# Amano-Ginji/distributed-tensorflow-example

Hardware: AMD Instinct MI355X
Metric: samples/sec (whole node) MNIST MLP sync-SGD at 1/2/4/8 MI355X; step-time p50 (higher is better)
Workload: dtype fp32; 1 GPU; model=mlp-784-100-10 (example.py), global_batch=100, per_gpu_batch=100, parallelism=dp1, optimizer=sgd lr=0.0005, grad_allreduce=none, engine=persistent-fp32, exchange_mode=persistent, launch=single process, steps_per_launch=550, hipgraph_steps=0, input_prefetch=in-kernel copier workgroups, activation=sigmoid

## Files before the change

csrc/kernels/mlp_persist_f32.hip:

```cpp
#include "common.h"
#include "mlp_api.h"

#include <atomic>

#include <cstdlib>

namespace dtfk {
namespace mlpf {

typedef __attribute__((ext_vector_type(4))) uint32_t u32x4;
typedef __attribute__((address_space(1))) unsigned gu32;

constexpr int DIN = 784, HID = 100, NCLS = 10;
constexpr int NJ = 7;
constexpr int NQ = 4;
constexpr int NTW = 2;
constexpr int NBT = 7;
constexpr int BROWS = 16 * NBT;
constexpr int XTS = 128;
constexpr int NCOMP = NJ * NQ;
constexpr int THREADS = 512;
constexpr int NCOP = 16;
constexpr int NCOPR = 14;
constexpr int RES_LR_BYTE = 124;
// ... 257 lines not shown
  f32x4 S0 = {0.f, 0.f, 0.f, 0.f}, S1 = S0;
#pragma unroll
  for (int r0 = 0; r0 < NW; r0 += GRP) {
    if (r0 >= W) break;
    u32x4 v0[GRP], v1[GRP];
#pragma unroll
    for (int i = 0; i < GRP; ++i) {
      const int r = r0 + i;
      const bool on = r < W && r != rank && hv;
      const auto rs = prs.r[r];
      if constexpr (BF) {
        if constexpr (TWO) {
          v0[i] = __builtin_amdgcn_raw_buffer_load_b128(rs, on ? so + e0 : OOB_OFF, 0, SYS);
        } else {
          const u32x2 h = __builtin_amdgcn_raw_buffer_load_b64(rs, on ? so + e0 : OOB_OFF, 0, SYS);
          v0[i] = u32x4{h[0], h[1], 0u, 0u};
        }
      } else {
        v0[i] = __builtin_amdgcn_raw_buffer_load_b128(rs, on ? so + e0 : OOB_OFF, 0, SYS);
        if constexpr (TWO) v1[i] = __builtin_amdgcn_raw_buffer_load_b128(rs, on ? so + e1 : OOB_OFF, 0, SYS);
      }
    }
#pragma unroll
    for (int i = 0; i < GRP; ++i) {
      const int r = r0 + i;
      if (r >= W) break;
      const bool me = r == rank;
      f32x4 P0, P1 = {0.f, 0.f, 0.f, 0.f};
      if constexpr (BF) {
        P0 = unbf4(v0[i][0], v0[i][1]);
        if constexpr (TWO) P1 = unbf4(v0[i][2], v0[i][3]);
      } else {
        P0 = __builtin_bit_cast(f32x4, v0[i]);
        if constexpr (TWO) P1 = __builtin_bit_cast(f32x4, v1[i]);
      }
      S0 += me ? G0 : P0;
      S1 += me ? G1 : P1;
    }
  }
  G0 = S0;
  G1 = S1;
}
template <int NW>
__device__ __forceinline__ void sum_small(const PeerRs<NW>& prs, int W, int rank, int so, bool dlane, bool blane,
                                          int lane, f32x4& D, float& gb) {
  u32x4 d[NW];
  uint32_t b[NW];
#pragma unroll
  for (int r = 0; r < NW; ++r) {
    const bool on = r < W && r != rank;
    const auto rs = prs.r[r];
    d[r] = __builtin_amdgcn_raw_buffer_load_b128(rs, (on && dlane) ? so + lane * 16 : OOB_OFF, 0, SYS);
    b[r] = __builtin_amdgcn_raw_buffer_load_b32(rs, (on && blane) ? so + 1024 + lane * 4 : OOB_OFF, 0, SYS);
  }
  f32x4 SD = {0.f, 0.f, 0.f, 0.f};
  float SB = 0.f;
#pragma unroll
  for (int r = 0; r < NW; ++r) {
    if (r >= W) break;
    const bool me = r == rank;
    SD += me ? D : __builtin_bit_cast(f32x4, d[r]);
    SB += me ? gb : __uint_as_float(b[r]);
  }
  D = SD;
  gb = SB;
}

__device__ void copier(const Args& a, int cid, uint8_t* smem) {
  const int tid = threadIdx.x;
  const int B = a.B;
  if (tid == 0) { PRO(NCOMP + cid, 0); }
  for (int st = cid; st < a.next_steps; st += NCOP) {
    const uint8_t* src = a.host_next + (long long)st * a.rec_h;
    uint8_t* dst = a.stage_next + (long long)st * REC;
    constexpr int C16 = DIN / 16;
    for (int k = tid; k < BROWS * C16; k += THREADS) {
      const int row = k / C16, c = k % C16;
      uint4 v = make_uint4(0u, 0u, 0u, 0u);
      if (row < B) v = reinterpret_cast<const uint4*>(src)[row * C16 + c];
      *reinterpret_cast<uint4*>(smem + row * CROW + 16 * c) = v;
    }
    if (tid < 128) dst[XROW_BYTES + XT_BYTES + tid] = tid < B ? src[(long long)B * DIN + tid] : (uint8_t)0;
    __syncthreads();
    for (int k = tid; k < BROWS * C16; k += THREADS) {
      const int row = k / C16, c = k % C16;
      reinterpret_cast<uint4*>(dst)[row * C16 + c] = *reinterpret_cast<const uint4*>(smem + row * CROW + 16 * c);
    }
    uint8_t* xt = dst + XROW_BYTES;
    for (int k = tid; k < (DIN / 4) * (BROWS / 4); k += THREADS) {
      const int fq = k / (BROWS / 4), rq = k % (BROWS / 4);
      const uint8_t* p = smem + 4 * rq * CROW + 4 * fq;
      const uint32_t r0 = *reinterpret_cast<const uint32_t*>(p);
      const uint32_t r1 = *reinterpret_cast<const uint32_t*>(p + CROW);
      const uint32_t r2 = *reinterpret_cast<const uint32_t*>(p + 2 * CROW);
      const uint32_t r3 = *reinterpret_cast<const uint32_t*>(p + 3 * CROW);
      const uint32_t t01 = __builtin_amdgcn_perm(r1, r0, 0x05010400u);
      const uint32_t t23 = __builtin_amdgcn_perm(r3, r2, 0x05010400u);
      const uint32_t u01 = __builtin_amdgcn_perm(r1, r0, 0x07030602u);
      const uint32_t u23 = __builtin_amdgcn_perm(r3, r2, 0x07030602u);
      uint32_t* o = reinterpret_cast<uint32_t*>(xt + (long long)(4 * fq) * XTS + 4 * rq);
      o[0] = __builtin_amdgcn_perm(t23, t01, 0x05040100u);
      o[XTS / 4] = __builtin_amdgcn_perm(t23, t01, 0x07060302u);
      o[2 * XTS / 4] = __builtin_amdgcn_perm(u23, u01, 0x05040100u);
      o[3 * XTS / 4] = __builtin_amdgcn_perm(u23, u01, 0x07060302u);
    }
    __syncthreads();
  }
  if (tid == 0) { PRO(NCOMP + cid, 1); }
}

__device__ void copier_res(const Args& a, int cid, uint8_t* smem) {
  if (cid >= NCOPR) return;
  const int tid = threadIdx.x;
  constexpr int RR = 8;
  int* dec = reinterpret_cast<int*>(smem + RR * CROW);
  const int B = a.B;
  const int hb = (int)(2 * a.rec_h);
  const auto hrs = __builtin_amdgcn_make_buffer_rsrc(const_cast<uint8_t*>(a.host_recs), 0, hb, 0x00020000);
  for (int st = 0;; ++st) {
    const long long k = a.run0 + st;
    if (tid == 0) {
      int d = 1;
      const long long t0 = (long long)__builtin_amdgcn_s_memrealtime();
      const long long lim = cid == 0 ? a.idle : a.idle + a.timeout;
      for (;;) {
        const long long v = __hip_atomic_load(a.door, __ATOMIC_RELAXED, __HIP_MEMORY_SCOPE_SYSTEM);
        if (v < 0) { d = 0; break; }
        if (v > k) break;
        if (cid != 0 && __hip_atomic_load(a.dctr + 16, __ATOMIC_RELAXED, __HIP_MEMORY_SCOPE_AGENT) != 0u) { d = 0; break; }
        if ((long long)__builtin_amdgcn_s_memrealtime() - t0 > lim) { d = 0; break; }
        __builtin_amdgcn_s_sleep(1);
      }
      if (cid == 0 && !d) __hip_atomic_store(a.dctr + 16, 1u, __ATOMIC_RELAXED, __HIP_MEMORY_SCOPE_AGENT);
      if (cid == 0 && d) { RTS(k, 0); }
      *dec = d;
    }
    __syncthreads();
    if (*dec == 0) break;
    const int slot = (int)(k & 1);
    const int hbase = slot * (int)a.rec_h;
    const int r0 = RR * cid;
    uint8_t* dst = const_cast<uint8_t*>(a.stage) + (long long)(st & 1) * REC;
    constexpr int C16 = DIN / 16;
    constexpr int NLD = (RR * C16 + THREADS - 1) / THREADS;
    u32x4 hv[NLD];
    uint32_t lv = 0;
    if (cid == 0 && tid < 32) {
      if (4 * tid == RES_LR_BYTE)
        lv = __float_as_uint(__hip_atomic_load(a.host_lr + slot, __ATOMIC_RELAXED, __HIP_MEMORY_SCOPE_SYSTEM));
      else
        lv = __builtin_amdgcn_raw_buffer_load_b32(hrs, 4 * tid < B ? hbase + B * DIN + 4 * tid : OOB_OFF, 0, SYS);
    }
#pragma unroll
    for (int i = 0; i < NLD; ++i) {
      const int t = tid + i * THREADS;
      const int rr = t / C16, cc = t % C16;
      const int row = r0 + rr;
      hv[i] = __builtin_amdgcn_raw_buffer_load_b128(hrs, (t < RR * C16 && row < B) ? hbase + row * DIN + 16 * cc : OOB_OFF,
                                                    0, SYS);
    }
#pragma unroll
    for (int i = 0; i < NLD; ++i) {
      const int t = tid + i * THREADS;
      if (t < RR * C16) *reinterpret_cast<u32x4*>(smem + (t / C16) * CROW + 16 * (t % C16)) = hv[i];
    }
    __syncthreads();
    for (int t = tid; t < RR * C16; t += THREADS) {
      const int rr = t / C16, cc = t % C16;
      const u32x4 v = *reinterpret_cast<const u32x4*>(smem + rr * CROW + 16 * cc);
      __builtin_amdgcn_raw_buffer_store_b128(v, region_rsrc(dst, (int)REC), (r0 + rr) * DIN + 16 * cc, 0, 16);
    }
    for (int t = tid; t < (DIN / 4) * (RR / 4); t += THREADS) {
      const int fq = t >> 1, rq = t & 1;
      const uint8_t* p = smem + 4 * rq * CROW + 4 * fq;
      const uint32_t q0 = *reinterpret_cast<const uint32_t*>(p);
      const uint32_t q1 = *reinterpret_cast<const uint32_t*>(p + CROW);
      const uint32_t q2 = *reinterpret_cast<const uint32_t*>(p + 2 * CROW);
      const uint32_t q3 = *reinterpret_cast<const uint32_t*>(p + 3 * CROW);
      const uint32_t t01 = __builtin_amdgcn_perm(q1, q0, 0x05010400u);
      const uint32_t t23 = __builtin_amdgcn_perm(q3, q2, 0x05010400u);
      const uint32_t u01 = __builtin_amdgcn_perm(q1, q0, 0x07030602u);
      const uint32_t u23 = __builtin_amdgcn_perm(q3, q2, 0x07030602u);
      const auto rs = region_rsrc(dst, (int)REC);
      const int o = (int)XROW_BYTES + (4 * fq) * XTS + r0 + 4 * rq;
      __builtin_amdgcn_raw_buffer_store_b32(__builtin_amdgcn_perm(t23, t01, 0x05040100u), rs, o, 0, 16);
      __builtin_amdgcn_raw_buffer_store_b32(__builtin_amdgcn_perm(t23, t01, 0x07060302u), rs, o + XTS, 0, 16);
      __builtin_amdgcn_raw_buffer_store_b32(__builtin_amdgcn_perm(u23, u01, 0x05040100u), rs, o + 2 * XTS, 0, 16);
      __builtin_amdgcn_raw_buffer_store_b32(__builtin_amdgcn_perm(u23, u01, 0x07060302u), rs, o + 3 * XTS, 0, 16);
    }
    if (cid == 0 && tid < 32) {
      uint32_t v = lv;
      if (4 * tid != RES_LR_BYTE) {
        const int nv = B - 4 * tid;
        if (nv < 4) v = nv <= 0 ? 0u : (v & ((1u << (8 * nv)) - 1u));
      }
      __builtin_amdgcn_raw_buffer_store_b32(v, region_rsrc(dst, (int)REC), (int)(XROW_BYTES + XT_BYTES) + 4 * tid, 0,
                                            16);
    }
    asm volatile("s_waitcnt vmcnt(0)" ::: "memory");
    __syncthreads();
    if (tid == 0) {
      __hip_atomic_fetch_add(a.dctr, 1u, __ATOMIC_RELAXED, __HIP_MEMORY_SCOPE_AGENT);
      if (cid == 0) { RTS(k, 1); }
    }
  }
  if (cid == 0 && tid == 0)
    __hip_atomic_store(a.host_state, a.launch_id, __ATOMIC_RELAXED, __HIP_MEMORY_SCOPE_SYSTEM);
}

template <int ACT, int NW, bool SPLIT, bool RES, bool INS = false>
__device__ void compute(const Args& a, const int j, const int q, uint8_t* smem) {
  const int dbg = INS ? a.dbg : 0;
  constexpr bool MULTI = NW > 1;
  const int tid = threadIdx.x, lane = tid & 63, w = __builtin_amdgcn_readfirstlane(tid >> 6);
  const int r = lane & 15, g = lane >> 4;
  const int c = j * NQ + q;
  const int B = a.B;
  f32x4* zbuf = reinterpret_cast<f32x4*>(smem + L_ZBUF);
  float* a2T = reinterpret_cast<float*>(smem + L_A2T);
  float* dz2T = reinterpret_cast<float*>(smem + L_DZ2T);
  float* dz3T = reinterpret_cast<float*>(smem + L_DZ3T);
  float* w2s = reinterpret_cast<float*>(smem + L_W2);
  float* b1s = reinterpret_cast<float*>(smem + L_B1);
  float* b2s = reinterpret_cast<float*>(smem + L_B2);
  float* rdb2 = reinterpret_cast<float*>(smem + L_RDB2);
  int* abort_flag = reinterpret_cast<int*>(smem + L_FLAG);
  int* census = abort_flag + 1;
  uint16_t* dzp = reinterpret_cast<uint16_t*>(smem + L_DZP);
  if (tid == 0) { PROC(c, 0); }

  const int hid = 16 * j + r;
  const bool hv = hid < HID;
  const int nt = ntile(q);
  const bool tv0 = w < nt, tv1 = w + 8 < nt;
  const int ft0 = tile0(q) + w, ft1 = tile0(q) + (tv1 ? w + 8 : 0);
  auto tvk = [=](int k) { return k ? tv1 : tv0; };
  auto ftk = [=](int k) { return k ? ft1 : ft0; };
  float Wt[NTW][4];
  f32x4 wld[NTW];
  if constexpr (RES) {
#pragma unroll
    for (int k = 0; k < NTW; ++k)
#pragma unroll
      for (int e = 0; e < 4; ++e)
        Wt[k][e] = (tvk(k) && hv) ? a.params[(16 * ftk(k) + 4 * g + e) * HID + hid] : 0.f;
  } else if constexpr (MULTI) {
    const int u0 = 16 * j + 4 * (r & 3);
#pragma unroll
    for (int k = 0; k < NTW; ++k)
      wld[k] = (tvk(k) && u0 < HID)
                   ? *reinterpret_cast<const f32x4*>(a.params + (16 * ftk(k) + 4 * g + (r >> 2)) * HID + u0)
                   : f32x4{0.f, 0.f, 0.f, 0.f};
  } else {
    const int u0 = 16 * j + 4 * (r & 3);
    const auto rw1 = __builtin_amdgcn_make_buffer_rsrc(a.params, 0, DIN * HID * 4, 0x00020000);
#pragma unroll
    for (int k = 0; k < NTW; ++k)
      wld[k] = __builtin_bit_cast(
          f32x4, __builtin_amdgcn_raw_buffer_load_b128(
                     rw1, (tvk(k) && u0 < HID) ? ((16 * ftk(k) + 4 * g + (r >> 2)) * HID + u0) * 4 : OOB_OFF, 0, 0));
  }
  float pv = 0.f;
  if constexpr (MULTI) {
    if (tid < 256) {
      const int n = tid >> 4, cl = tid & 15;
      const int hn = 16 * j + n;
      pv = (hn < HID && cl < NCLS) ? a.p_w2[hn * NCLS + cl] : 0.f;
    } else if (tid < 272) {
      const int hn = 16 * j + (tid - 256);
      pv = hn < HID ? a.p_b1[hn] : 0.f;
    } else if (tid < 288) {
      const int cl = tid - 272;
      pv = cl < NCLS ? a.p_b2[cl] : 0.f;
    }
  } else {
    const int n = tid >> 4, cl = tid & 15, hn = 16 * j + n, hb = 16 * j + (tid - 256), c2 = tid - 272;
    const auto rw2 = __builtin_amdgcn_make_buffer_rsrc(a.p_w2, 0, HID * NCLS * 4, 0x00020000);
    const auto rb1 = __builtin_amdgcn_make_buffer_rsrc(a.p_b1, 0, HID * 4, 0x00020000);
    const auto rb2 = __builtin_amdgcn_make_buffer_rsrc(a.p_b2, 0, NCLS * 4, 0x00020000);
    const uint32_t v0 =
        __builtin_amdgcn_raw_buffer_load_b32(rw2, (tid < 256 && hn < HID && cl < NCLS) ? (hn * NCLS + cl) * 4 : OOB_OFF, 0, 0);
    const uint32_t v1 =
        __builtin_amdgcn_raw_buffer_load_b32(rb1, (tid >= 256 && tid < 272 && hb < HID) ? hb * 4 : OOB_OFF, 0, 0);
    const uint32_t v2 =
        __builtin_amdgcn_raw_buffer_load_b32(rb2, (tid >= 272 && tid < 288 && c2 < NCLS) ? c2 * 4 : OOB_OFF, 0, 0);
    pv = __uint_as_float(v0 | v1 | v2);
  }
  unsigned long long seq0 = *a.seq;
  long long gstep0 = *a.gstep;
  float lr = *a.lr;
  const unsigned xcc = __builtin_amdgcn_s_getreg((15 << 11) | (0 << 6) | 20) & 15u;
  unsigned long long* hdr = reinterpret_cast<unsigned long long*>(a.xbuf + HDR_OFF);
  const unsigned tag0 = a.census_tag;
  if (tid == 0)
    __hip_atomic_store(hdr + c, ((unsigned long long)tag0 << 32) | xcc, __ATOMIC_RELAXED, __HIP_MEMORY_SCOPE_AGENT);
  for (int k = tid; k < 3 * 16 * LS; k += THREADS) a2T[k] = 0.f;
  if constexpr (SPLIT)
    for (int k = tid; k < 3 * 16 * PS; k += THREADS) dzp[k] = (uint16_t)0;
  const bool failed_in = __hip_atomic_load(a.err, __ATOMIC_RELAXED, __HIP_MEMORY_SCOPE_AGENT) != 0;

  constexpr int XTN = SPLIT ? 8 : NBT;
  uint32_t xf[NTW][NBT], xt[NTW][XTN];
  int lab = 0;
  auto tlk = [=](int k) { return k ? (tv1 ? w + 8 : 0) : w; };
  auto stage_x = [&](int st, int n0, int dn) {
    const uint8_t* rec = a.stage + (long long)st * REC;
    const uint8_t* xr = rec + 16 * tile0(q);
#pragma unroll 1
    for (int n = n0; n < (XF_CHUNKS + 63) / 64; n += dn) {
      const int k = 64 * n + lane;
      if (k < XF_CHUNKS) glds16(xr + (k / 13) * DIN + 16 * (k % 13), smem + L_XF + 1024 * n);
    }
    const uint8_t* xtb = rec + XROW_BYTES + (long long)(16 * tile0(q)) * XTS;
#pragma unroll 1
    for (int n = n0; n < XT_CHUNKS / 64; n += dn) {
      const int f = 8 * n + (lane >> 3);
      const int s = (lane & 7) ^ ((f >> 1) & 7);
      if (f < 16 * nt) glds16(xtb + f * XTS + 16 * s, smem + L_XT + 1024 * n);
    }
    if (n0 == 0 && lane < 8) glds16(rec + XROW_BYTES + XT_BYTES + 16 * lane, smem + L_LAB);
  };
  auto read_xf = [&]() {
#pragma unroll
    for (int k = 0; k < NTW; ++k)
#pragma unroll
      for (int b = 0; b < NBT; ++b)
        xf[k][b] = *reinterpret_cast<const uint32_t*>(smem + L_XF + (16 * b + r) * XF_ROW + 16 * tlk(k) + 4 * g);
    lab = smem[L_LAB + 16 * (w < NBT ? w : NBT - 1) + r];
  };
  auto read_xt = [&]() {
#pragma unroll
    for (int k = 0; k < NTW; ++k) {
      const int f = 16 * tlk(k) + r;
      if constexpr (SPLIT) {
#pragma unroll
        for (int cc = 0; cc < 4; ++cc) {
          const uint2 v = *reinterpret_cast<const uint2*>(
              smem + L_XT + f * XTS + 16 * ((2 * cc + (g >> 1)) ^ ((f >> 1) & 7)) + 8 * (g & 1));
          xt[k][2 * cc] = v.x;
          xt[k][2 * cc + 1] = v.y;
        }
      } else {
#pragma unroll
        for (int s = 0; s < NBT; ++s)
          xt[k][s] = *reinterpret_cast<const uint32_t*>(smem + L_XT + f * XTS + 16 * (s ^ ((f >> 1) & 7)) + 4 * g);
      }
    }
  };
  if (tid == 0) { PROC(c, 4); }
  if constexpr (!RES) stage_x(0, w, 8);
  if (w == 0) {
    const long long t0 = (long long)__builtin_amdgcn_s_memrealtime();
    unsigned long long v = 0;
    bool seen = lane >= NCOMP, bad = false;
    for (;;) {
      if (!seen) {
        v = __hip_atomic_load(hdr + lane, __ATOMIC_RELAXED, __HIP_MEMORY_SCOPE_AGENT);
        seen = (unsigned)(v >> 32) == tag0;
      }
      if (__all(seen)) break;
      if ((long long)__builtin_amdgcn_s_memrealtime() - t0 > a.timeout) {
        if (lane == 0) atomicOr(a.err, 1);
        bad = true;
        break;
      }
      __builtin_amdgcn_s_sleep(1);
    }
    const bool off = lane < NCOMP && (unsigned)v != xcc;
    const bool e1 = !__any(off && lane / NQ == j);
    const bool e2 = !__any(off && lane % NQ == q);
    if (lane == 0) *census = bad ? -1 : ((e1 ? 1 : 0) | (e2 ? 2 : 0));
  }
  if (tid < 256) {
    w2s[tid] = pv;
  } else if (tid < 272) {
    b1s[tid - 256] = pv;
  } else if (tid < 288) {
    b2s[tid - 272] = pv;
  } else if (tid == 288) {
    *abort_flag = 0;
  } else if (tid >= 296 && tid < 304) {
    reinterpret_cast<int*>(smem + L_HFLAG)[tid - 296] = 0;
  }
  asm volatile("s_waitcnt vmcnt(0)" ::: "memory");
  if constexpr (!MULTI) {
    asm volatile("" : "+v"(seq0), "+v"(gstep0), "+v"(lr));
    seq0 = ((unsigned long long)__builtin_amdgcn_readfirstlane((unsigned)(seq0 >> 32)) << 32) |
           __builtin_amdgcn_readfirstlane((unsigned)seq0);
    gstep0 = (long long)(((unsigned long long)__builtin_amdgcn_readfirstlane((unsigned)((unsigned long long)gstep0 >> 32))
                          << 32) |
                         __builtin_amdgcn_readfirstlane((unsigned)gstep0));
  }
  double gvar0 = 0.0;
  if constexpr (RES) {
    if (a.gvar_kind == 1) gvar0 = *static_cast<const float*>(a.gvar);
    else if (a.gvar_kind == 2) gvar0 = (double)*static_cast<const long long*>(a.gvar);
    else if (a.gvar_kind == 3) gvar0 = *static_cast<const int*>(a.gvar);
    else if (a.gvar_kind == 4) gvar0 = *static_cast<const double*>(a.gvar);
    else gvar0 = (double)gstep0;
  }
#pragma unroll
  for (int k = 0; k < NTW && !RES; ++k) {
    const int m = r & 3, b = r >> 2;
#pragma unroll
    for (int t = 0; t < 4; ++t) {
      const int cs = (b + t) & 3;
      const float v = cs == 0 ? wld[k][0] : (cs == 1 ? wld[k][1] : (cs == 2 ? wld[k][2] : wld[k][3]));
      const int e = (m - t) & 3;
      const float got = __shfl(v, 16 * g + 4 * e + b);
#pragma unroll
      for (int q = 0; q < 4; ++q)
        if (q == e) Wt[k][q] = got;
    }
  }
  __syncthreads();
  float lrB = lr / (float)(B * (MULTI ? a.W : 1));
  float lrX = lrB * (1.f / 255.f);
  if (failed_in || *census < 0) return;
  const bool l2_e1 = (*census & 1) != 0;
  const bool l2_e2 = (*census & 2) != 0;
  if (tid == 0) { PROC(c, 1); }
  if constexpr (!RES) {
    read_xf();
    read_xt();
  }
  if (tid == 0) { PROC(c, 2); }

  auto res_stage = [&](int st) -> bool {
    int* rflag = abort_flag + 2;
    if (tid == 0) {
      const unsigned need = (unsigned)NCOPR * (unsigned)(st + 1);
      const long long t0 = (long long)__builtin_amdgcn_s_memrealtime();
      int v = 1;
      for (;;) {
        if (__hip_atomic_load(a.dctr, __ATOMIC_RELAXED, __HIP_MEMORY_SCOPE_AGENT) >= need) break;
        if (__hip_atomic_load(a.dctr + 16, __ATOMIC_RELAXED, __HIP_MEMORY_SCOPE_AGENT) != 0u) { v = 0; break; }
        if ((long long)__builtin_amdgcn_s_memrealtime() - t0 > a.idle + a.timeout) {
          atomicOr(a.err, 4);
          v = 0;
          break;
        }
        __builtin_amdgcn_s_sleep(1);
      }
      *rflag = v;
    }
    __syncthreads();
    if (*rflag == 0) return false;
    if (c == 0 && tid == 0) { RTSC(a.run0 + st, 2); }
    const auto rs = region_rsrc(a.stage + (long long)(st & 1) * REC, (int)REC);
    const int xr0 = 16 * tile0(q);
#pragma unroll 4
    for (int k = tid; k < XF_CHUNKS; k += THREADS) {
      const u32x4 v = __builtin_amdgcn_raw_buffer_load_b128(rs, (k / 13) * DIN + 16 * (k % 13) + xr0, 0, 16);
      *reinterpret_cast<u32x4*>(smem + L_XF + 16 * k) = v;
    }
    const int xt0 = (int)XROW_BYTES + 16 * tile0(q) * XTS;
#pragma unroll 4
    for (int k = tid; k < XT_CHUNKS; k += THREADS) {
      const int f = k >> 3;
      if (f < 16 * nt) {
        const int sw = (k & 7) ^ ((f >> 1) & 7);
        const u32x4 v = __builtin_amdgcn_raw_buffer_load_b128(rs, xt0 + f * XTS + 16 * sw, 0, 16);
        *reinterpret_cast<u32x4*>(smem + L_XT + 16 * k) = v;
      }
    }
    if (tid < 8) {
      const u32x4 v = __builtin_amdgcn_raw_buffer_load_b128(rs, (int)(XROW_BYTES + XT_BYTES) + 16 * tid, 0, 16);
      *reinterpret_cast<u32x4*>(smem + L_LAB + 16 * tid) = v;
    }
    __syncthreads();
    read_xf();
    read_xt();
    if (c == 0 && tid == 0) { RTSC(a.run0 + st, 3); }
    const float lr_run = *reinterpret_cast<const float*>(smem + L_LAB + RES_LR_BYTE);
    lrB = lr_run / (float)B;
    lrX = lrB * (1.f / 255.f);
    return true;
  };
  int st_done = 0;
  auto write_params = [&](bool wt) {
    auto put = [wt](float* p, float v) {
      if (wt) __hip_atomic_store(p, v, __ATOMIC_RELAXED, __HIP_MEMORY_SCOPE_AGENT);
      else *p = v;
    };
    if (hv) {
#pragma unroll
      for (int k = 0; k < NTW; ++k)
        if (tvk(k)) {
#pragma unroll
          for (int e = 0; e < 4; ++e) put(a.params + (16 * ftk(k) + 4 * g + e) * HID + hid, Wt[k][e]);
        }
    }
    if (q == 0) {
      if (tid < 256) {
        const int n = tid >> 4, cl = tid & 15;
        const int hn = 16 * j + n;
        if (hn < HID && cl < NCLS) put(a.p_w2 + hn * NCLS + cl, w2s[tid]);
      } else if (tid < 272) {
        const int hn = 16 * j + (tid - 256);
        if (hn < HID) put(a.p_b1 + hn, b1s[tid - 256]);
      }
    }
    if (c == 0 && tid >= 272 && tid < 272 + NCLS) put(a.p_b2 + (tid - 272), b2s[tid - 272]);
  };

  const PeerRs<NW> prs = peer_rsrcs<NW>(a.peer_base, MULTI ? a.W : 1);
  bool aborted = false;
  for (int st = 0; st < a.nsteps; ++st) {
    if constexpr (RES) {
      if (!res_stage(st)) break;
    }
    int jq[2] = {j, q};
    asm volatile("" : "+s"(jq[0]), "+s"(jq[1]));
    const unsigned long long sq = seq0 + (unsigned long long)st + 1ull;
    const unsigned tag = (unsigned)sq;
    const int par = (int)(sq & 1ull);
    if (c == 0 && tid == 0 && a.step_ts != nullptr)
      a.step_ts[(gstep0 + st) % a.ts_ring] = (long long)__builtin_amdgcn_s_memrealtime();
    if (w == 0) { PH(0); }
    if (w == 7) { PH7(14); }

    {
      f32x4 acc[NBT];
#pragma unroll
      for (int b = 0; b < NBT; ++b) acc[b] = f32x4{0.f, 0.f, 0.f, 0.f};
      if constexpr (SPLIT) {
        float wv[8];
#pragma unroll
        for (int i = 0; i < 8; ++i) wv[i] = Wt[i >> 2][i & 3];
        bf16x8 Ah, Am, Al;
        split8(wv, Ah, Am, Al);
        bf16x8 X[NBT];
#pragma unroll
        for (int b = 0; b < NBT; ++b) X[b] = px8(xf[0][b], xf[1][b]);
#pragma unroll
        for (int b = 0; b < NBT; ++b) acc[b] = mfma16x16x32(Al, X[b], acc[b]);
#pragma unroll
        for (int b = 0; b < NBT; ++b) acc[b] = mfma16x16x32(Am, X[b], acc[b]);
#pragma unroll
        for (int b = 0; b < NBT; ++b) acc[b] = mfma16x16x32(Ah, X[b], acc[b]);
      } else {
#pragma unroll
        for (int k = 0; k < NTW; ++k) {
          if (tvk(k)) {
#pragma unroll
            for (int e = 0; e < 4; ++e)
#pragma unroll
              for (int b = 0; b < NBT; ++b) acc[b] = mfma4(Wt[k][e], ub(xf[k][b], e), acc[b]);
          }
        }
      }
#pragma unroll
      for (int b = 0; b < NBT; ++b) zbuf[(w * NBT + b) * 64 + lane] = acc[b];
    }
    if (w == 0) { PH(1); }
    lds_barrier();
    if (w == 0) { PH(2); }
    const bool more = !RES && st + 1 < a.nsteps;
    int* hflag = reinterpret_cast<int*>(smem + L_HFLAG);
    auto heads_done = [&]() -> unsigned {
      const bool ok = lane < NBT && __hip_atomic_load(hflag + (lane < NBT ? lane : 0), __ATOMIC_RELAXED,
                                                      __HIP_MEMORY_SCOPE_WORKGROUP) >= st + 1;
      return (unsigned)__ballot(ok) & ((1u << NBT) - 1u);
    };
    if (w == 7 && more && !(dbg & 1)) {
      stage_x(st + 1, 0, 1);
      asm volatile("s_waitcnt vmcnt(0)" ::: "memory");
      __builtin_amdgcn_fence(__ATOMIC_RELEASE, "workgroup", "local");
      if (lane == 0) __hip_atomic_store(hflag + 7, st + 1, __ATOMIC_RELAXED, __HIP_MEMORY_SCOPE_WORKGROUP);
    } else if (w == 7 && more && lane == 0) {
      __hip_atomic_store(hflag + 7, st + 1, __ATOMIC_RELAXED, __HIP_MEMORY_SCOPE_WORKGROUP);
    }

    if (w < NBT) {
      const int bw = 16 * w + r;
      const bool bv = bw < B;
      f32x4 zs = zbuf[w * 64 + lane];
#pragma unroll
      for (int v = 1; v < 8; ++v) zs += zbuf[(v * NBT + w) * 64 + lane];
      const auto r1 = region_rsrc(a.xbuf + E1_OFF + (long long)(par * NJ + j) * NQ * NBT * GSLOT, NQ * NBT * GSLOT);
      put_gran(r1, (q * NBT + w) * GSLOT + 32 * lane, zs, tag, l2_e1);
      if (w == 0) { PH(3); }
      float w2p[4], w2d[4], b1v[4], b2v[4];
#pragma unroll
      for (int e = 0; e < 4; ++e) {
        w2p[e] = w2s[(4 * g + e) * 16 + r];
        w2d[e] = w2s[r * 16 + 4 * g + e];
        b1v[e] = b1s[4 * g + e];
        b2v[e] = b2s[4 * g + e];
      }
      f32x4 part[NQ];
      bool ok = gather_gran<NQ>(r1, [&](int k) { return (k * NBT + w) * GSLOT; }, jq[1], true, tag, zs, part, lane, a);
      f32x4 z = part[0];
#pragma unroll
      for (int qq = 1; qq < NQ; ++qq) z += part[qq];
      if (w == 0) { PH(4); }
      if (w == 0) { PH(5); }
      float a2[4];
#pragma unroll
      for (int i = 0; i < 4; ++i) {
        const int hl = 4 * g + i;
        const float zt = z[i] * (1.f / 255.f) + b1v[i];
        const float av = ACT == 0 ? __builtin_amdgcn_rcpf(1.f + __expf(-zt)) : fmaxf(zt, 0.f);
        a2[i] = (16 * j + hl < HID) ? av : 0.f;
      }
      f32x4 pl = {0.f, 0.f, 0.f, 0.f};
#pragma unroll
      for (int e = 0; e < 4; ++e) pl = mfma4(w2p[e], a2[e], pl);
      const auto r2 = region_rsrc(a.xbuf + E2_OFF + (long long)((par * NQ + q) * NBT + w) * NJ * GSLOT, NJ * GSLOT);
      if (g < 3) put_gran(r2, j * GSLOT + 32 * lane, pl, tag, l2_e2);
      if (w == 0) { PH(6); }
#pragma unroll
      for (int i = 0; i < 4; ++i) a2T[(4 * g + i) * LS + bw] = a2[i];
      f32x4 lp[NJ];
      ok = gather_gran<NJ>(r2, [&](int k) { return k * GSLOT; }, jq[0], g < 3, tag, pl, lp, lane, a) && ok;
      if (w == 0) { PH(7); }
      if (!ok && lane == 0) *abort_flag = 1;
      float lg[4], ex[4];
      float m = -3.0e38f;
#pragma unroll
      for (int i = 0; i < 4; ++i) {
        float v = b2v[i];
#pragma unroll
        for (int jj = 0; jj < NJ; ++jj) v += lp[jj][i];
        lg[i] = v;
        if (4 * g + i < NCLS) m = fmaxf(m, v);
      }
      if (w == 0) { PH(8); }
      m = fmaxf(m, xor16(m));
      m = fmaxf(m, xor32(m));
      const int y = lab < NCLS ? lab : 0;
      float ssum = 0.f, zy = 0.f, am = 1e9f;
#pragma unroll
      for (int i = 0; i < 4; ++i) {
        const int cl = 4 * g + i;
        ex[i] = cl < NCLS ? __expf(lg[i] - m) : 0.f;
        ssum += ex[i];
        zy += (cl == y) ? lg[i] : 0.f;
        if (cl < NCLS && lg[i] == m) am = fminf(am, (float)cl);
      }
      ssum += xor16(ssum); ssum += xor32(ssum);
      zy += xor16(zy); zy += xor32(zy);
      am = fminf(am, xor16(am)); am = fminf(am, xor32(am));
      const float inv = __builtin_amdgcn_rcpf(ssum);
      if (w == 0) { PHX(13); }
      float dz3[4], py = 0.f;
#pragma unroll
      for (int i = 0; i < 4; ++i) {
        const int cl = 4 * g + i;
        const float p = ex[i] * inv;
        py += (cl == y) ? p : 0.f;
        dz3[i] = (bv && cl < NCLS) ? p - (cl == y ? 1.f : 0.f) : 0.f;
      }
      py += xor16(py); py += xor32(py);
      const float loss = a.naive ? -__logf(py) : (m + __logf(ssum) - zy);
      f32x4 da = {0.f, 0.f, 0.f, 0.f};
#pragma unroll
      for (int e = 0; e < 4; ++e) da = mfma4(w2d[e], dz3[e], da);
      if (w == 0) { PHX(14); }
#pragma unroll
      for (int i = 0; i < 4; ++i) {
        const float d = ACT == 0 ? da[i] * a2[i] * (1.f - a2[i]) : (a2[i] > 0.f ? da[i] : 0.f);
        if constexpr (SPLIT) {
          uint32_t ph, pm, pl;
          split3(d, ph, pm, pl);
          const int o = (4 * g + i) * PS + bw;
          dzp[o] = (uint16_t)(ph >> 16);
          dzp[16 * PS + o] = (uint16_t)(pm >> 16);
          dzp[32 * PS + o] = (uint16_t)(pl >> 16);
        } else {
          dz2T[(4 * g + i) * LS + bw] = d;
        }
        dz3T[(4 * g + i) * LS + bw] = dz3[i];
      }
      if (w == 0) { PHX(15); }
      if (g == 0) {
        float* rl = reinterpret_cast<float*>(smem + L_RLOSS);
        rl[bw] = bv ? loss : 0.f;
        rl[128 + bw] = (bv && (int)am == y) ? 1.f : 0.f;
      }
      asm volatile("s_waitcnt lgkmcnt(0)" ::: "memory");
      {
        const f32x4 av = *reinterpret_cast<const f32x4*>(a2T + r * LS + 16 * w + 4 * g);
        const f32x4 dv = *reinterpret_cast<const f32x4*>(dz3T + r * LS + 16 * w + 4 * g);
        const float one = r == 0 ? 1.f : 0.f;
        f32x4 dp = {0.f, 0.f, 0.f, 0.f}, p2 = dp;
#pragma unroll
        for (int e = 0; e < 4; ++e) {
          dp = mfma4(av[e], dv[e], dp);
          p2 = mfma4(one, dv[e], p2);
        }
        reinterpret_cast<f32x4*>(smem + L_DW2P)[w * 64 + lane] = dp;
        if (g == 0) rdb2[w * 16 + r] = p2[0];
      }
      __builtin_amdgcn_fence(__ATOMIC_RELEASE, "workgroup", "local");
      if (lane == 0)
        __hip_atomic_store(reinterpret_cast<int*>(smem + L_HFLAG) + w, st + 1, __ATOMIC_RELAXED,
                           __HIP_MEMORY_SCOPE_WORKGROUP);
      if (w == 0) { PH(9); }
    }
    f32x4 G[NTW];
    f32x4 G1[NTW];
#pragma unroll
    for (int k = 0; k < NTW; ++k) G[k] = G1[k] = f32x4{0.f, 0.f, 0.f, 0.f};
    constexpr int NCH = SPLIT ? 4 : NBT;
    auto need_of = [](int ch) -> unsigned {
      return SPLIT ? ((1u << (2 * ch)) | (2 * ch + 1 < NBT ? 1u << (2 * ch + 1) : 0u)) : (1u << ch);
    };
    auto chunk = [&](int ch) {
      if constexpr (SPLIT) {
        const uint16_t* bp = dzp + r * PS + 32 * ch + 8 * g;
        const bf16x8 Bh = *reinterpret_cast<const bf16x8*>(bp);
        const bf16x8 Bm = *reinterpret_cast<const bf16x8*>(bp + 16 * PS);
        const bf16x8 Bl = *reinterpret_cast<const bf16x8*>(bp + 32 * PS);
        const bf16x8 X0 = px8(xt[0][2 * ch], xt[0][2 * ch + 1]);
        if (tv1 || w == 7) {
          const bf16x8 X1 = tv1 ? px8(xt[1][2 * ch], xt[1][2 * ch + 1]) : px8(0x01010101u, 0x01010101u);
          G[0] = mfma16x16x32(X0, Bl, G[0]);
          G[1] = mfma16x16x32(X1, Bl, G[1]);
          G[0] = mfma16x16x32(X0, Bm, G[0]);
          G[1] = mfma16x16x32(X1, Bm, G[1]);
          G[0] = mfma16x16x32(X0, Bh, G[0]);
          G[1] = mfma16x16x32(X1, Bh, G[1]);
        } else {
          G[0] = mfma16x16x32(X0, Bl, G[0]);
          G[0] = mfma16x16x32(X0, Bm, G[0]);
          G[0] = mfma16x16x32(X0, Bh, G[0]);
        }
      } else {
        const f32x4 bz = *reinterpret_cast<const f32x4*>(dz2T + r * LS + 16 * ch + 4 * g);
#pragma unroll
        for (int k = 0; k < NTW; ++k) {
          if (tvk(k)) {
            G[k] = mfma4(ub(xt[k][ch], 0), bz[0], G[k]);
            G1[k] = mfma4(ub(xt[k][ch], 1), bz[1], G1[k]);
            G[k] = mfma4(ub(xt[k][ch], 2), bz[2], G[k]);
            G1[k] = mfma4(ub(xt[k][ch], 3), bz[3], G1[k]);
          }
        }
        if (w == 7) {
          G[1] = mfma4(1.f, bz[0], G[1]);
          G1[1] = mfma4(1.f, bz[1], G1[1]);
          G[1] = mfma4(1.f, bz[2], G[1]);
          G1[1] = mfma4(1.f, bz[3], G1[1]);
        }
      }
    };
    {
      int cc = 0;
      for (;;) {
        const unsigned hm = heads_done();
        bool did = false;
#pragma unroll
        for (int ch = 0; ch < NCH; ++ch) {
          if (ch == cc && (hm & need_of(ch)) == need_of(ch)) {
            if (!did) __builtin_amdgcn_fence(__ATOMIC_ACQUIRE, "workgroup", "local");
            if (cc == 0 && w == 0) { PH(10); }
            chunk(ch);
            ++cc;
            did = true;
          }
        }
        if (cc == NCH) break;
        if (!did) __builtin_amdgcn_s_sleep(0);
      }
    }
    if constexpr (!SPLIT) {
#pragma unroll
      for (int k = 0; k < NTW; ++k) G[k] = G[k] + G1[k];
    }
    f32x4 D = {0.f, 0.f, 0.f, 0.f};
    float gb = 0.f;
    if (w == 7) {
      const float* gsrc = rdb2 + (lane >= 16 && lane < 16 + NCLS ? lane - 16 : 0);
      const f32x4* dw2p = reinterpret_cast<const f32x4*>(smem + L_DW2P);
#pragma unroll
      for (int v = 0; v < NBT; ++v) {
        D += dw2p[v * 64 + lane];
        gb += gsrc[v * 16];
      }
      if (lane < 16) gb = G[1][0];
      if (lane >= 16 + NCLS) gb = 0.f;
      PH7(13);
      PH7(15);
      if (c == 0) {
        const float* rl = reinterpret_cast<const float*>(smem + L_RLOSS);
        const bool hi = lane + 64 < BROWS;
        const float ls = wave_sum(rl[lane] + (hi ? rl[lane + 64] : 0.f));
        const float cr = wave_sum(rl[128 + lane] + (hi ? rl[128 + lane + 64] : 0.f));
        if (lane == 63) {
          const int sl = (int)((gstep0 + st) % a.ring);
          if constexpr (RES) {
            reinterpret_cast<float*>(abort_flag)[4] = ls / (float)B;
            reinterpret_cast<float*>(abort_flag)[5] = cr / (float)B;
            __hip_atomic_store(a.metrics + 2 * sl, ls / (float)B, __ATOMIC_RELAXED, __HIP_MEMORY_SCOPE_AGENT);
            __hip_atomic_store(a.metrics + 2 * sl + 1, cr / (float)B, __ATOMIC_RELAXED, __HIP_MEMORY_SCOPE_AGENT);
          } else {
            a.metrics[2 * sl] = ls / (float)B;
            a.metrics[2 * sl + 1] = cr / (float)B;
          }
        }
      }
      if constexpr (!MULTI) {
#pragma unroll
        for (int i = 0; i < 4; ++i)
          if (16 * j + 4 * g + i < HID && r < NCLS) w2s[(4 * g + i) * 16 + r] -= lrB * D[i];
        if (lane < 16) {
          if (16 * j + lane < HID) b1s[lane] -= lrB * gb;
        } else if (lane < 16 + NCLS) {
          b2s[lane - 16] -= lrB * gb;
        }
      }
    }
    if (*abort_flag) { aborted = true; break; }
    if (more) {
      while (__hip_atomic_load(hflag + 7, __ATOMIC_RELAXED, __HIP_MEMORY_SCOPE_WORKGROUP) < st + 1)
        __builtin_amdgcn_s_sleep(1);
      __builtin_amdgcn_fence(__ATOMIC_ACQUIRE, "workgroup", "local");
      read_xf();
      read_xt();
    }
    if (w == 0) { PH(11); }
    if constexpr (MULTI) {
      const bool pk = a.gbf16 != 0;
      const size_t soff = IPC_FLAGS + (size_t)(par * NCOMP + c) * IPC_SLOT;
      char* own = static_cast<char*>(a.peer_base[a.rank]) + soff;
      const int eb = (w * 64 + lane) * 16;
      const int ef0 = ((w * NTW + 0) * 64 + lane) * 16;
      const int ef1 = ((w * NTW + 1) * 64 + lane) * 16;
      const bool dlane = r < NCLS && 16 * j + 4 * g < HID;
      const bool blane = lane < 16 ? 16 * j + lane < HID : lane < 16 + NCLS;
      if (hv) {
        if (pk) {
          const uint32_t p0 = pack2bf(G[0][0], G[0][1]), p1 = pack2bf(G[0][2], G[0][3]);
          const uint32_t p2 = pack2bf(G[1][0], G[1][1]), p3 = pack2bf(G[1][2], G[1][3]);
          if (tv1) *reinterpret_cast<uint4*>(own + eb) = make_uint4(p0, p1, p2, p3);
          else if (tv0) *reinterpret_cast<uint2*>(own + eb) = make_uint2(p0, p1);
        } else {
          if (tv0) *reinterpret_cast<f32x4*>(own + ef0) = G[0];
          if (tv1) *reinterpret_cast<f32x4*>(own + ef1) = G[1];
        }
      }
      if (pk) {
        G[0] = round_bf16x4(G[0]);
        G[1] = round_bf16x4(G[1]);
      }
      if (w == 7) {
        if (dlane) *reinterpret_cast<f32x4*>(own + IPC_SMALL + lane * 16) = D;
        if (blane) *reinterpret_cast<float*>(own + IPC_SMALL + 1024 + lane * 4) = gb;
      }
      asm volatile("s_waitcnt vmcnt(0)" ::: "memory");
      lds_barrier();
      char* flags = static_cast<char*>(a.peer_base[a.rank]);
      auto wait_peers = [&](int fo) {
        if (w == 0) {
          const long long t0 = (long long)__builtin_amdgcn_s_memrealtime();
          for (;;) {
            bool ok = true;
            if (lane < a.W && lane != a.rank) {
              const unsigned v = __hip_atomic_load(
                  reinterpret_cast<const unsigned*>(static_cast<const char*>(a.peer_base[lane]) + 64 * c + fo),
                  __ATOMIC_RELAXED, __HIP_MEMORY_SCOPE_SYSTEM);
              ok = (int)(v - tag) >= 0;
            }
            if (__all(ok)) break;
            if ((long long)__builtin_amdgcn_s_memrealtime() - t0 > a.timeout ||
                __hip_atomic_load(a.err, __ATOMIC_RELAXED, __HIP_MEMORY_SCOPE_AGENT) != 0) {
              if (lane == 0) {
                atomicOr(a.err, 2);
                *abort_flag = 1;
              }
              break;
            }
            __builtin_amdgcn_s_sleep(1);
          }
        }
        lds_barrier();
        asm volatile("" ::: "memory");
      };
      if (tid == 0 && !(a.rank == a.fault_rank && gstep0 + st >= a.fault_step))
        __hip_atomic_store(reinterpret_cast<unsigned*>(flags + 64 * c), tag, __ATOMIC_RELAXED,
                           __HIP_MEMORY_SCOPE_SYSTEM);
      wait_peers(0);
      if (*abort_flag) { aborted = true; break; }
      auto sum_ranks = [&](size_t so) {
        constexpr int GF = NW < 4 ? NW : 4;
        if (pk) {
          if (tv1) sum_entries<NW, NW, true, true>(prs, a.W, a.rank, (int)so, hv, eb, eb, G[0], G[1]);
          else sum_entries<NW, NW, true, false>(prs, a.W, a.rank, (int)so, hv, eb, eb, G[0], G[1]);
        } else {
          if (tv1) sum_entries<NW, GF, false, true>(prs, a.W, a.rank, (int)so, hv, ef0, ef1, G[0], G[1]);
          else sum_entries<NW, GF, false, false>(prs, a.W, a.rank, (int)so, hv, ef0, ef1, G[0], G[1]);
        }
        if (w == 7) sum_small<NW>(prs, a.W, a.rank, (int)so + IPC_SMALL, dlane, blane, lane, D, gb);
      };
      if (a.xmode == 0) {
        sum_ranks(soff);
      } else {
        const int own_chunk = w % a.W;
        const size_t roff = IPC_RED + (size_t)(par * NCOMP + c) * IPC_SLOT;
        char* ored = static_cast<char*>(a.peer_base[a.rank]) + roff;
        if (own_chunk == a.rank) {
          sum_ranks(soff);
          if (hv) {
            if (pk) {
              const uint32_t p0 = pack2bf(G[0][0], G[0][1]), p1 = pack2bf(G[0][2], G[0][3]);
              const uint32_t p2 = pack2bf(G[1][0], G[1][1]), p3 = pack2bf(G[1][2], G[1][3]);
              if (tv1) *reinterpret_cast<uint4*>(ored + eb) = make_uint4(p0, p1, p2, p3);
              else if (tv0) *reinterpret_cast<uint2*>(ored + eb) = make_uint2(p0, p1);
              G[0] = round_bf16x4(G[0]);
              G[1] = round_bf16x4(G[1]);
            } else {
              if (tv0) *reinterpret_cast<f32x4*>(ored + ef0) = G[0];
              if (tv1) *reinterpret_cast<f32x4*>(ored + ef1) = G[1];
            }
          }
          if (w == 7) {
            if (dlane) *reinterpret_cast<f32x4*>(ored + IPC_SMALL + lane * 16) = D;
            if (blane) *reinterpret_cast<float*>(ored + IPC_SMALL + 1024 + lane * 4) = gb;
          }
        }
        asm volatile("s_waitcnt vmcnt(0)" ::: "memory");
        lds_barrier();
        if (tid == 0)
          __hip_atomic_store(reinterpret_cast<unsigned*>(flags + 64 * c + 8), tag, __ATOMIC_RELAXED,
                             __HIP_MEMORY_SCOPE_SYSTEM);
        wait_peers(8);
        if (*abort_flag) { aborted = true; break; }
        if (own_chunk != a.rank) {
          __amdgpu_buffer_rsrc_t rs = prs.r[0];
#pragma unroll
          for (int rr = 1; rr < NW; ++rr)
            if (rr == own_chunk) rs = prs.r[rr];
          const int ro = (int)roff;
          if (pk) {
            if (tv1) {
              const u32x4 v = __builtin_amdgcn_raw_buffer_load_b128(rs, hv ? ro + eb : OOB_OFF, 0, SYS);
              G[0] = unbf4(v[0], v[1]);
              G[1] = unbf4(v[2], v[3]);
            } else {
              const u32x2 v = __builtin_amdgcn_raw_buffer_load_b64(rs, hv ? ro + eb : OOB_OFF, 0, SYS);
              G[0] = unbf4(v[0], v[1]);
            }
          } else {
            G[0] = __builtin_bit_cast(f32x4, __builtin_amdgcn_raw_buffer_load_b128(rs, hv ? ro + ef0 : OOB_OFF, 0, SYS));
            if (tv1)
              G[1] = __builtin_bit_cast(f32x4, __builtin_amdgcn_raw_buffer_load_b128(rs, hv ? ro + ef1 : OOB_OFF, 0, SYS));
          }
          if (w == 7) {
            D = __builtin_bit_cast(
                f32x4, __builtin_amdgcn_raw_buffer_load_b128(rs, dlane ? ro + IPC_SMALL + lane * 16 : OOB_OFF, 0, SYS));
            gb = __uint_as_float(
                __builtin_amdgcn_raw_buffer_load_b32(rs, blane ? ro + IPC_SMALL + 1024 + lane * 4 : OOB_OFF, 0, SYS));
          }
        }
      }
    }
    if (hv) {
#pragma unroll
      for (int k = 0; k < NTW; ++k)
#pragma unroll
        for (int i = 0; i < 4; ++i) Wt[k][i] -= (k == 0 || tv1) ? lrX * G[k][i] : 0.f;
    }
    if (w == 0) { PH(12); }
    if (MULTI && w == 7) {
#pragma unroll
      for (int i = 0; i < 4; ++i)
        if (16 * j + 4 * g + i < HID && r < NCLS) w2s[(4 * g + i) * 16 + r] -= lrB * D[i];
      if (lane < 16) {
        if (16 * j + lane < HID) b1s[lane] -= lrB * gb;
      } else if (lane < 16 + NCLS) {
        b2s[lane - 16] -= lrB * gb;
      }
    }
    st_done = st + 1;
    if constexpr (RES) {
      __syncthreads();
      if (c == 0 && tid == 0) { RTSC(a.run0 + st, 4); }
      write_params(true);
      const double gsv = gvar0 + (double)(st + 1);
      if (c == 0 && tid == 0) {
        if (a.gvar_kind == 1) __hip_atomic_store(static_cast<float*>(a.gvar), (float)gsv, __ATOMIC_RELAXED, __HIP_MEMORY_SCOPE_AGENT);
        else if (a.gvar_kind == 2) __hip_atomic_store(static_cast<long long*>(a.gvar), (long long)gsv, __ATOMIC_RELAXED, __HIP_MEMORY_SCOPE_AGENT);
        else if (a.gvar_kind == 3) __hip_atomic_store(static_cast<int*>(a.gvar), (int)gsv, __ATOMIC_RELAXED, __HIP_MEMORY_SCOPE_AGENT);
        else if (a.gvar_kind == 4) __hip_atomic_store(static_cast<double*>(a.gvar), gsv, __ATOMIC_RELAXED, __HIP_MEMORY_SCOPE_AGENT);
      }
      asm volatile("s_waitcnt vmcnt(0)" ::: "memory");
      __syncthreads();
      if (tid == 0) {
        if (c == 0) { RTSC(a.run0 + st, 5); }
        __hip_atomic_fetch_add(a.dctr + 32, 1u, __ATOMIC_RELAXED, __HIP_MEMORY_SCOPE_AGENT);
        if (c == 0) {
          const unsigned need = (unsigned)NCOMP * (unsigned)(st + 1);
          const long long t0 = (long long)__builtin_amdgcn_s_memrealtime();
          while (__hip_atomic_load(a.dctr + 32, __ATOMIC_RELAXED, __HIP_MEMORY_SCOPE_AGENT) < need) {
            if ((long long)__builtin_amdgcn_s_memrealtime() - t0 > a.timeout) {
              atomicOr(a.err, 8);
              break;
            }
          }
          RTSC(a.run0 + st, 6);
          const float* mf = reinterpret_cast<const float*>(abort_flag);
          __hip_atomic_store(a.host_out, mf[4], __ATOMIC_RELAXED, __HIP_MEMORY_SCOPE_SYSTEM);
          __hip_atomic_store(a.host_out + 1, mf[5], __ATOMIC_RELAXED, __HIP_MEMORY_SCOPE_SYSTEM);
          __hip_atomic_store(a.host_out + 2, (float)gsv, __ATOMIC_RELAXED, __HIP_MEMORY_SCOPE_SYSTEM);
          asm volatile("s_waitcnt vmcnt(0)" ::: "memory");
          __hip_atomic_store(a.host_done, a.run0 + st + 1, __ATOMIC_RELAXED, __HIP_MEMORY_SCOPE_SYSTEM);
          RTSC(a.run0 + st, 7);
        }
      }
    }
  }
  if (aborted) return;
  __syncthreads();
  if (tid == 0) { PROC(c, 3); }

  write_params(false);
  if (c == 0 && tid == 300) {
    *a.gstep = gstep0 + st_done;
    *a.seq = seq0 + (unsigned long long)st_done;
    if (a.step_ts != nullptr)
      a.step_ts[(gstep0 + st_done) % a.ts_ring] = (long long)__builtin_amdgcn_s_memrealtime();
  }
  if (tid == 0) { PROC(c, 5); }
}

template <int ACT, int NW, bool SPLIT, bool RES = false, bool INS = false>
__global__ __launch_bounds__(THREADS, 1) void mlp_persist_f32(Args a) {
  extern __shared__ __attribute__((aligned(16))) uint8_t smem[];
  const int b = blockIdx.x;
  int c = -1, cid = -1;
  if (a.spread) {
    if (b < NCOMP) c = b; else cid = b - NCOMP;
  } else {
    if ((b & 7) == 0) c = b >> 3; else cid = b - (b >> 3) - 1;
  }
  if (c >= 0) {
    if (a.nsteps > 0) compute<ACT, NW, SPLIT, RES, INS>(a, c / NQ, c % NQ, smem);
    return;
  }
  if constexpr (RES) copier_res(a, cid, smem);
  else if (cid < NCOP) copier(a, cid, smem);
}

static int g_fault_rank = -1;
static long long g_fault_step = -1;

static unsigned next_census_tag() {
  static std::atomic<unsigned> ctr{0};
  unsigned t = ctr.fetch_add(1u, std::memory_order_relaxed) + 1u;
  return t == 0u ? ctr.fetch_add(1u, std::memory_order_relaxed) + 1u : t;
}

static int persist_dbg() {
  static const int dbg = [] {
    const char* db = getenv("DTF_PERSIST_DBG");
    return db ? atoi(db) : 0;
  }();
  return dbg;
}

static Args make_args(const Launch& p) {
  const bool res = p.door != nullptr;
  Args a{};
  a.stage = static_cast<const uint8_t*>(p.stage);
  a.rec_h = p.rec_h;
  a.B = p.B;
  a.nsteps = res ? 0x7fffffff : p.nsteps;
  a.params = p.params;
  a.lr = p.lr;
  a.metrics = p.metrics;
  a.ring = p.ring;
  a.act = p.act;
  a.naive = p.naive;
  a.gstep = p.gstep;
  a.seq = p.seq;
  a.xbuf = static_cast<uint8_t*>(p.xbuf);
  a.err = p.err;
  a.timeout = p.timeout;
  a.step_ts = p.step_ts;
  a.ts_ring = p.ts_ring > 0 ? p.ts_ring : 1;
  a.host_next = static_cast<const uint8_t*>(p.host_next);
  a.next_steps = p.next_steps;
  a.stage_next = static_cast<uint8_t*>(p.stage_next);
  a.peer_base = p.peer_base;
  a.W = p.W;
  a.rank = p.rank;
  a.gbf16 = p.gbf16;
  a.spread = p.spread;
  a.phase_ts = p.phase_ts;
  a.xmode = p.xmode;
  a.fault_step = g_fault_step;
  a.fault_rank = g_fault_rank;
  a.p_w2 = p.W2 != nullptr ? p.W2 : p.params + OFF_W2;
  a.p_b1 = p.b1 != nullptr ? p.b1 : p.params + OFF_B1;
  a.p_b2 = p.b2 != nullptr ? p.b2 : p.params + OFF_B2;
  a.door = p.door;
  a.host_recs = static_cast<const uint8_t*>(p.host_recs);
  a.host_lr = p.host_lr;
  a.host_out = p.host_out;
  a.host_done = p.host_done;
  a.host_state = p.host_state;
  a.launch_id = p.launch_id;
  a.run0 = p.run0;
  a.idle = p.idle;
  a.census_tag = next_census_tag();
  a.gvar = p.gvar;
  a.gvar_kind = p.gvar_kind;
  a.dctr = p.dctr;
  a.res_ts = p.res_ts;
  a.dbg = res ? 0 : persist_dbg();
  return a;
}

typedef void (*Kern)(Args);
static const Kern kKernels[24] = {
    mlp_persist_f32<0, 1, false>, mlp_persist_f32<1, 1, false>, mlp_persist_f32<0, 2, false>,
    mlp_persist_f32<1, 2, false>, mlp_persist_f32<0, 4, false>, mlp_persist_f32<1, 4, false>,
    mlp_persist_f32<0, 8, false>, mlp_persist_f32<1, 8, false>, mlp_persist_f32<0, 1, true>,
    mlp_persist_f32<1, 1, true>,  mlp_persist_f32<0, 2, true>,  mlp_persist_f32<1, 2, true>,
    mlp_persist_f32<0, 4, true>,  mlp_persist_f32<1, 4, true>,  mlp_persist_f32<0, 8, true>,
    mlp_persist_f32<1, 8, true>,
    mlp_persist_f32<0, 1, false, false, true>, mlp_persist_f32<1, 1, false, false, true>,
    mlp_persist_f32<0, 1, true, false, true>,  mlp_persist_f32<1, 1, true, false, true>,
// ... 53 lines not shown
```

Measured before the change: 13.90 million samples/s.

## Pre-pack bf16 input fragments and prefetch next-step inputs early on wave 7

In the split-bf16, non-resident, single-worker path, input fragments are packed into bf16x8 registers once per step (forward XF and backward XA) instead of re-packing inside the MFMA loops. Wave 7 also packs its backward operands and loads the next step's inputs right after signalling the stage flag, so that read moves off the step tail. The cost is more live vector registers and a loop-carried label variable (lab_n). Empty asm pins stop the compiler from rematerializing the packs.

```diff
diff --git a/csrc/kernels/mlp_persist_f32.hip b/csrc/kernels/mlp_persist_f32.hip
--- a/csrc/kernels/mlp_persist_f32.hip
+++ b/csrc/kernels/mlp_persist_f32.hip
@@ -583,6 +583,14 @@
   constexpr int XTN = SPLIT ? 8 : NBT;
   uint32_t xf[NTW][NBT], xt[NTW][XTN];
   int lab = 0;
+  constexpr bool PREP = SPLIT && !RES && NW == 1;
+  bf16x8 XF[NBT], XA[NTW][4];
+  int lab_n = 0;
+  auto pin8 = [](bf16x8& v) {
+    u32x4 t = __builtin_bit_cast(u32x4, v);
+    asm volatile("" : "+v"(t));
+    v = __builtin_bit_cast(bf16x8, t);
+  };
   auto tlk = [=](int k) { return k ? (tv1 ? w + 8 : 0) : w; };
   auto stage_x = [&](int st, int n0, int dn) {
     const uint8_t* rec = a.stage + (long long)st * REC;
@@ -601,13 +609,13 @@
     }
     if (n0 == 0 && lane < 8) glds16(rec + XROW_BYTES + XT_BYTES + 16 * lane, smem + L_LAB);
   };
-  auto read_xf = [&]() {
+  auto read_xf = [&](int& lb) {
 #pragma unroll
     for (int k = 0; k < NTW; ++k)
 #pragma unroll
       for (int b = 0; b < NBT; ++b)
         xf[k][b] = *reinterpret_cast<const uint32_t*>(smem + L_XF + (16 * b + r) * XF_ROW + 16 * tlk(k) + 4 * g);
-    lab = smem[L_LAB + 16 * (w < NBT ? w : NBT - 1) + r];
+    lb = smem[L_LAB + 16 * (w < NBT ? w : NBT - 1) + r];
   };
   auto read_xt = [&]() {
 #pragma unroll
@@ -626,6 +634,31 @@
         for (int s = 0; s < NBT; ++s)
           xt[k][s] = *reinterpret_cast<const uint32_t*>(smem + L_XT + f * XTS + 16 * (s ^ ((f >> 1) & 7)) + 4 * g);
       }
+    }
+  };
+  auto prep_fwd = [&](int& lb) {
+    read_xf(lb);
+#pragma unroll
+    for (int b = 0; b < NBT; ++b) XF[b] = px8(xf[0][b], xf[1][b]);
+#pragma unroll
+    for (int b = 0; b < NBT; ++b) pin8(XF[b]);
+    read_xt();
+  };
+  auto prep_xa = [&]() {
+    if constexpr (SPLIT) {
+#pragma unroll
+      for (int k = 0; k < NTW; ++k)
+#pragma unroll
+        for (int i = 0; i < 8; ++i) asm volatile("" : "+v"(xt[k][i]));
+#pragma unroll
+      for (int ch = 0; ch < 4; ++ch) {
+        XA[0][ch] = px8(xt[0][2 * ch], xt[0][2 * ch + 1]);
+        XA[1][ch] = tv1 ? px8(xt[1][2 * ch], xt[1][2 * ch + 1]) : px8(0x01010101u, 0x01010101u);
+      }
+#pragma unroll
+      for (int k = 0; k < NTW; ++k)
+#pragma unroll
+        for (int ch = 0; ch < 4; ++ch) pin8(XA[k][ch]);
     }
   };
   if (tid == 0) { PROC(c, 4); }
@@ -701,8 +734,10 @@
   const bool l2_e1 = (*census & 1) != 0;
   const bool l2_e2 = (*census & 2) != 0;
   if (tid == 0) { PROC(c, 1); }
-  if constexpr (!RES) {
-    read_xf();
+  if constexpr (PREP) {
+    prep_fwd(lab);
+  } else if constexpr (!RES) {
+    read_xf(lab);
     read_xt();
   }
   if (tid == 0) { PROC(c, 2); }
@@ -750,7 +785,7 @@
       *reinterpret_cast<u32x4*>(smem + L_LAB + 16 * tid) = v;
     }
     __syncthreads();
-    read_xf();
+    read_xf(lab);
     read_xt();
     if (c == 0 && tid == 0) { RTSC(a.run0 + st, 3); }
     const float lr_run = *reinterpret_cast<const float*>(smem + L_LAB + RES_LR_BYTE);
@@ -813,7 +848,10 @@
         split8(wv, Ah, Am, Al);
         bf16x8 X[NBT];
 #pragma unroll
-        for (int b = 0; b < NBT; ++b) X[b] = px8(xf[0][b], xf[1][b]);
+        for (int b = 0; b < NBT; ++b) {
+          if constexpr (PREP) X[b] = XF[b];
+          else X[b] = px8(xf[0][b], xf[1][b]);
+        }
 #pragma unroll
         for (int b = 0; b < NBT; ++b) acc[b] = mfma16x16x32(Al, X[b], acc[b]);
 #pragma unroll
@@ -849,8 +887,20 @@
       asm volatile("s_waitcnt vmcnt(0)" ::: "memory");
       __builtin_amdgcn_fence(__ATOMIC_RELEASE, "workgroup", "local");
       if (lane == 0) __hip_atomic_store(hflag + 7, st + 1, __ATOMIC_RELAXED, __HIP_MEMORY_SCOPE_WORKGROUP);
+      PH7(15);
     } else if (w == 7 && more && lane == 0) {
       __hip_atomic_store(hflag + 7, st + 1, __ATOMIC_RELAXED, __HIP_MEMORY_SCOPE_WORKGROUP);
+    }
+    bool prepped = false;
+    if constexpr (PREP) {
+      if (w == 7) {
+        prep_xa();
+        if (more && !(dbg & 4)) {
+          __builtin_amdgcn_fence(__ATOMIC_ACQUIRE, "workgroup", "local");
+          prep_fwd(lab_n);
+          prepped = true;
+        }
+      }
     }
 
     if (w < NBT) {
@@ -862,6 +912,7 @@
       const auto r1 = region_rsrc(a.xbuf + E1_OFF + (long long)(par * NJ + j) * NQ * NBT * GSLOT, NQ * NBT * GSLOT);
       put_gran(r1, (q * NBT + w) * GSLOT + 32 * lane, zs, tag, l2_e1);
       if (w == 0) { PH(3); }
+      if constexpr (PREP) prep_xa();
       float w2p[4], w2d[4], b1v[4], b2v[4];
 #pragma unroll
       for (int e = 0; e < 4; ++e) {
@@ -994,9 +1045,12 @@
         const bf16x8 Bh = *reinterpret_cast<const bf16x8*>(bp);
         const bf16x8 Bm = *reinterpret_cast<const bf16x8*>(bp + 16 * PS);
         const bf16x8 Bl = *reinterpret_cast<const bf16x8*>(bp + 32 * PS);
-        const bf16x8 X0 = px8(xt[0][2 * ch], xt[0][2 * ch + 1]);
+        bf16x8 X0, X1;
+        if constexpr (PREP) X0 = XA[0][ch];
+        else X0 = px8(xt[0][2 * ch], xt[0][2 * ch + 1]);
         if (tv1 || w == 7) {
-          const bf16x8 X1 = tv1 ? px8(xt[1][2 * ch], xt[1][2 * ch + 1]) : px8(0x01010101u, 0x01010101u);
+          if constexpr (PREP) X1 = XA[1][ch];
+          else X1 = tv1 ? px8(xt[1][2 * ch], xt[1][2 * ch + 1]) : px8(0x01010101u, 0x01010101u);
           G[0] = mfma16x16x32(X0, Bl, G[0]);
           G[1] = mfma16x16x32(X1, Bl, G[1]);
           G[0] = mfma16x16x32(X0, Bm, G[0]);
@@ -1063,7 +1117,6 @@
       if (lane < 16) gb = G[1][0];
       if (lane >= 16 + NCLS) gb = 0.f;
       PH7(13);
-      PH7(15);
       if (c == 0) {
         const float* rl = reinterpret_cast<const float*>(smem + L_RLOSS);
         const bool hi = lane + 64 < BROWS;
@@ -1094,13 +1147,18 @@
       }
     }
     if (*abort_flag) { aborted = true; break; }
-    if (more) {
+    if (more && !prepped) {
       while (__hip_atomic_load(hflag + 7, __ATOMIC_RELAXED, __HIP_MEMORY_SCOPE_WORKGROUP) < st + 1)
         __builtin_amdgcn_s_sleep(1);
       __builtin_amdgcn_fence(__ATOMIC_ACQUIRE, "workgroup", "local");
-      read_xf();
-      read_xt();
-    }
+      if constexpr (PREP) {
+        prep_fwd(lab_n);
+      } else {
+        read_xf(lab);
+        read_xt();
+      }
+    }
+    if constexpr (PREP) lab = lab_n;
     if (w == 0) { PH(11); }
     if constexpr (MULTI) {
       const bool pk = a.gbf16 != 0;
```

Result: faster. 14.52 million samples/s, median of 6 (+4.4%).
